# jhultman/vision3d

Measured on AMD Instinct MI355X. Metric: frames/sec SECOND fwd, 16k-pt KITTI cloud, higher is better.
Workload: dtype f16x3-scaled (fp32-class): fp32 operands split into f16 hi + lo pieces of x * s under per-tensor power-of-two scales, 3 MFMA terms (lo*hi + hi*lo + hi*hi), fp32 accumulate; relative product error 2^-22 -- the result differs from the reference's fp32 modules by fp32 summation noise: strict elementwis

## Files before the change

### vision3d_amd/csrc/spconv.hip

```cpp
#include "v3d_internal.h"

#include "sp_device.h"
#include "rb_device.h"

#define SP_RIDER_PROLOGUE(lds)                                                                        \
  if (rider.blocks && (int)blockIdx.x < rider.blocks) {                                               \
    if (threadIdx.x < V3D_BLOCK) rb_rider_run(rider, (int)blockIdx.x, (unsigned char*)(lds));         \
    return;                                                                                           \
  }                                                                                                   \
  const int bid = (int)blockIdx.x - rider.blocks;                                                     \
  [[maybe_unused]] const int nblk = (int)gridDim.x - rider.blocks;



__global__ __launch_bounds__(V3D_BLOCK) void spconv_fwd_scalar(const float* __restrict__ in,
                                                               const float* __restrict__ W,
                                                               const int* __restrict__ nbr,
                                                               const int* __restrict__ n_ptr, int cap, int K, int Cin,
                                                               int Cout, const float* __restrict__ scale,
                                                               const float* __restrict__ shift, int relu,
                                                               float* __restrict__ out) {
  const int n = min(*n_ptr, cap);
  const long long total = (long long)n * Cout;
  for (long long t = (long long)blockIdx.x * V3D_BLOCK + threadIdx.x; t < total; t += (long long)gridDim.x * V3D_BLOCK) {
    const int o = (int)(t / Cout), c = (int)(t % Cout);
    float acc = 0.f;
    for (int k = 0; k < K; k++) {
      const int i = nbr[(size_t)k * cap + o];
      if (i < 0) continue;
      const float* x = in + (size_t)i * Cin;
      const float* w = W + (size_t)k * Cin * Cout + c;
      float part = 0.f;
      for (int ci = 0; ci < Cin; ci++) part = fmaf(x[ci], w[(size_t)ci * Cout], part);
      acc += part;
    }
    if (scale) acc = acc * scale[c] + shift[c];
    if (relu) acc = fmaxf(acc, 0.f);
    out[t] = acc;
  }
}

#define SPC_TM 64

#define SPW_WAVES 8

template <int CIN, int COUT>
__global__ __launch_bounds__(SPW_WAVES* V3D_WAVE) void spconv_fwd_wave(const float* __restrict__ in,
                                                                       const float* __restrict__ W,
                                                                       const int* __restrict__ nbr,
                                                                       const int* __restrict__ n_ptr, int cap, int K,
                                                                       const float* __restrict__ scale,
                                                                       const float* __restrict__ shift, int relu,
                                                                       float* __restrict__ out, const float* __restrict__ next_entry,
                                                                       int* __restrict__ range_flag, unsigned* __restrict__ seen,
                                                                       const RbScanJob rider) {
  constexpr int NB = COUT / 16;
  constexpr int G = SPW_WAVES / NB;
  constexpr int T = CIN / 4;
  constexpr int NT = SPW_WAVES * V3D_WAVE;
  extern __shared__ __attribute__((aligned(16))) float smem[];
  float* acc = smem;
  int* list_in = (int*)(acc + G * SPC_TM * COUT);
  int* cnt_pad = list_in + K * SPC_TM;
  unsigned char* list_row = (unsigned char*)(cnt_pad + K);
  SP_RIDER_PROLOGUE(smem)

  const int n = min(*n_ptr, cap);
  const int row0 = bid * SPC_TM;
  if (row0 >= n) return;
  const int tid = threadIdx.x, lane = tid & 63, wave = tid >> 6;

  for (int i = tid; i < G * SPC_TM * COUT; i += NT) acc[i] = 0.f;
  for (int k = wave; k < K; k += SPW_WAVES) {
    const int row = row0 + lane;
    const int v = row < n ? nbr[(size_t)k * cap + row] : -1;
    const unsigned long long m = __ballot(v >= 0);
    const int c = __popcll(m);
    const int cp = (c + 15) & ~15;
    const int pos = __popcll(m & ((1ull << lane) - 1ull));
    if (v >= 0) {
      list_in[k * SPC_TM + pos] = v;
      list_row[k * SPC_TM + pos] = (unsigned char)lane;
    }
    if (lane >= c && lane < cp) {
      list_in[k * SPC_TM + lane] = -1;
      list_row[k * SPC_TM + lane] = 255;
    }
    if (lane == 0) cnt_pad[k] = cp;
  }
  __syncthreads();

  const int uwave = __builtin_amdgcn_readfirstlane(wave);
  const int g = uwave / NB, nb = uwave % NB;
  const int kper = (K + G - 1) / G;
  const int k_lo = g * kper, k_hi = min(K, k_lo + kper);
  const int r = lane & 15, q = lane >> 4;
  float* my_acc = acc + (size_t)g * SPC_TM * COUT + nb * 16 + r;
  const int cnt_reg = lane < K ? cnt_pad[lane] : 0;
  auto count_of = [&](int k) { return __builtin_amdgcn_readlane(cnt_reg, k); };

  float a0[T], a1[T], b0[T], b1[T];
  auto load_a = [&](int k, int rblk, float (&a)[T]) {
    const int src = list_in[k * SPC_TM + rblk * 16 + r];
    if (src >= 0) {
      const float* p = in + (size_t)src * CIN + q * T;
      if constexpr (T % 4 == 0) {
#pragma unroll
        for (int i = 0; i < T / 4; i++) {
          const float4 v = reinterpret_cast<const float4*>(p)[i];
          a[4 * i] = v.x;
          a[4 * i + 1] = v.y;
          a[4 * i + 2] = v.z;
          a[4 * i + 3] = v.w;
        }
      } else {
#pragma unroll
        for (int t = 0; t < T; t++) a[t] = p[t];
      }
    } else {
#pragma unroll
      for (int t = 0; t < T; t++) a[t] = 0.f;
    }
  };
  auto load_b = [&](int k, float (&b)[T]) {
    const float* p = W + ((size_t)k * CIN + q * T) * COUT + nb * 16 + r;
#pragma unroll
    for (int t = 0; t < T; t++) b[t] = p[(size_t)t * COUT];
  };
  auto advance = [&](int& k, int& rblk) {
    rblk++;
    if (rblk * 16 < count_of(k)) return;
    rblk = 0;
    do {
      k++;
    } while (k < k_hi && count_of(k) == 0);
  };

  int k = k_lo, rblk = 0;
  while (k < k_hi && count_of(k) == 0) k++;
  if (k < k_hi) {
    load_a(k, rblk, a0);
    load_b(k, b0);
  }
  while (k < k_hi) {
    int kn = k, rn = rblk;
    advance(kn, rn);
    const bool more = kn < k_hi, newk = kn != k;
    const unsigned rows4 = *reinterpret_cast<const unsigned*>(list_row + k * SPC_TM + rblk * 16 + q * 4);
    if (more) {
      load_a(kn, rn, a1);
      if (newk) load_b(kn, b1);
    }
    f32x4 d0 = {0.f, 0.f, 0.f, 0.f}, d1 = {0.f, 0.f, 0.f, 0.f};
    if constexpr (T >= 2) {
#pragma unroll
      for (int t = 0; t < T; t += 2) {
        d0 = __builtin_amdgcn_mfma_f32_16x16x4f32(a0[t], b0[t], d0, 0, 0, 0);
        d1 = __builtin_amdgcn_mfma_f32_16x16x4f32(a0[t + 1], b0[t + 1], d1, 0, 0, 0);
      }
      d0 += d1;
    } else {
      d0 = __builtin_amdgcn_mfma_f32_16x16x4f32(a0[0], b0[0], d0, 0, 0, 0);
    }
    {
      float old[4];
#pragma unroll
      for (int rr = 0; rr < 4; rr++) {
        const unsigned trow = (rows4 >> (8 * rr)) & 255u;
        old[rr] = trow != 255u ? my_acc[trow * COUT] : 0.f;
      }
#pragma unroll
      for (int rr = 0; rr < 4; rr++) {
        const unsigned trow = (rows4 >> (8 * rr)) & 255u;
        if (trow != 255u) my_acc[trow * COUT] = old[rr] + d0[rr];
      }
    }
    if (more) {
#pragma unroll
      for (int t = 0; t < T; t++) a0[t] = a1[t];
      if (newk) {
#pragma unroll
        for (int t = 0; t < T; t++) b0[t] = b1[t];
      }
    }
    k = kn;
    rblk = rn;
  }
  __syncthreads();

  float vmax = 0.f;
  for (int idx = tid; idx < SPC_TM * (COUT / 4); idx += NT) {
    const int rw = idx / (COUT / 4), c4 = idx % (COUT / 4);
    if (row0 + rw >= n) continue;
    float4 v = *reinterpret_cast<const float4*>(acc + rw * COUT + c4 * 4);
#pragma unroll
    for (int gg = 1; gg < G; gg++) {
      const float4 u = *reinterpret_cast<const float4*>(acc + ((size_t)gg * SPC_TM + rw) * COUT + c4 * 4);
      v.x += u.x;
      v.y += u.y;
      v.z += u.z;
      v.w += u.w;
    }
    if (scale) {
      const float4 sc = *reinterpret_cast<const float4*>(scale + c4 * 4);
      const float4 sh = *reinterpret_cast<const float4*>(shift + c4 * 4);
      v.x = v.x * sc.x + sh.x;
      v.y = v.y * sc.y + sh.y;
      v.z = v.z * sc.z + sh.z;
      v.w = v.w * sc.w + sh.w;
    }
    if (relu) {
      v.x = fmaxf(v.x, 0.f);
      v.y = fmaxf(v.y, 0.f);
      v.z = fmaxf(v.z, 0.f);
      v.w = fmaxf(v.w, 0.f);
    }
    vmax = fmaxf(fmaxf(vmax, fmaxf(fabsf(v.x), fabsf(v.y))), fmaxf(fabsf(v.z), fabsf(v.w)));
    *reinterpret_cast<float4*>(out + (size_t)(row0 + rw) * COUT + c4 * 4) = v;
  }
  if (next_entry && range_flag && vmax > next_entry[2]) atomicMax(range_flag, V3D_FLAG_RANGE);
  if (seen && next_entry) v3d_mark_seen(seen, vmax, next_entry[2] * (1.f / (float)(1 << V3D_QUIET_BITS)));
}

template <int CIN, int COUT>
static int launch_wave(const float* in, const float* W, const int* nbr, const int* n_ptr, int cap, int K,
                       const float* scale, const float* shift, int relu, float* out, hipStream_t st, const float* next_entry,
                       int* range_flag, unsigned* seen, const RbScanJob* rider, bool* rider_taken) {
  constexpr int G = SPW_WAVES / (COUT / 16);
  const size_t lds = std::max((size_t)G * SPC_TM * COUT * 4 + (size_t)K * SPC_TM * 4 + (size_t)K * 4 + (size_t)K * SPC_TM + 64, (size_t)RB_SCAN_LDS);
  if (lds > 64 * 1024) return V3D_EUNSUPPORTED;
  const RbScanJob r = rider ? *rider : RbScanJob{};
  hipLaunchKernelGGL((spconv_fwd_wave<CIN, COUT>), dim3(v3d_ceil_div(cap, SPC_TM) + r.blocks), dim3(SPW_WAVES * V3D_WAVE), lds, st,
                     in, W, nbr, n_ptr, cap, K, scale, shift, relu, out, next_entry, range_flag, seen, r);
  if (rider_taken) *rider_taken = r.blocks > 0;
  V3D_CHECK_LAUNCH();
  return V3D_OK;
}


template <int PREC>
__global__ void spconv_pack_weights_kernel(const float* __restrict__ W, int K, int Cin, int Cout, unsigned short* __restrict__ img) {
  const int KI = (Cin + 31) / 32, NB = Cout / 16;
  const long long total = (long long)K * KI * NB * 64 * 8;
  float sw = 1.f;
  if constexpr (PREC == 1) sw = v3d_wimg_weight_scale(reinterpret_cast<unsigned*>(img + total * 2));
  for (long long t = (long long)blockIdx.x * blockDim.x + threadIdx.x; t < total; t += (long long)gridDim.x * blockDim.x) {
    long long r = t;
    const int e = (int)(r % 8); r /= 8;
    const int lane = (int)(r % 64); r /= 64;
    const int nb = (int)(r % NB); r /= NB;
    const int ki = (int)(r % KI); r /= KI;
    const int k = (int)r;
    const int cin = ki * 32 + (lane >> 4) * 8 + e, cout = nb * 16 + (lane & 15);
    const float v = cin < Cin ? W[((size_t)k * Cin + cin) * Cout + cout] : 0.f;
    unsigned short h, l;
    split_one<PREC>(v, sw, h, l);
    const size_t base = ((((size_t)k * KI + ki) * NB + nb) * 2) * 512 + (size_t)lane * 8 + e;
    img[base] = h;
    img[base + 512] = l;
  }
}

__global__ void spconv_pack_batch_kernel(V3dPackJobs jobs) {
  const int j = blockIdx.y;
  const float* __restrict__ W = jobs.w[j];
  unsigned short* __restrict__ img = reinterpret_cast<unsigned short*>(jobs.img[j]);
  const int K = jobs.K[j], Cin = jobs.cin[j], Cout = jobs.cout[j], mode = jobs.mode[j];
  const int KI = (Cin + 31) / 32, NB = Cout / 16;
  const long long total = (long long)K * KI * NB * 64 * 8;
  for (long long t = (long long)blockIdx.x * blockDim.x + threadIdx.x; t < total; t += (long long)gridDim.x * blockDim.x) {
    long long r = t;
    const int e = (int)(r % 8); r /= 8;
    const int lane = (int)(r % 64); r /= 64;
    const int nb = (int)(r % NB); r /= NB;
    const int ki = (int)(r % KI); r /= KI;
    const int k = (int)r;
    const int cin = ki * 32 + (lane >> 4) * 8 + e, cout = nb * 16 + (lane & 15);
    float v = 0.f;
    if (cin < Cin) {
      if (mode == 0) v = W[((size_t)k * Cin + cin) * Cout + cout];
      else v = W[((size_t)(mode == 2 ? K - 1 - k : k) * Cout + cout) * Cin + cin];
    }
    unsigned short h, l;
    split_one<0>(v, 1.f, h, l);
    const size_t base = ((((size_t)k * KI + ki) * NB + nb) * 2) * 512 + (size_t)lane * 8 + e;
    img[base] = h;
    img[base + 512] = l;
  }
}

int v3d_i_sparse_conv_pack_batch(const V3dPackJobs& jobs, int n, hipStream_t stream) {
  if (n < 1 || n > V3D_PACK_JOBS_MAX) return V3D_EINVAL;
  for (int j = 0; j < n; j++)
    if (!jobs.w[j] || !jobs.img[j] || jobs.K[j] < 1 || jobs.cin[j] < 1 || jobs.cout[j] < 16 || jobs.cout[j] % 16) return V3D_EINVAL;
  hipLaunchKernelGGL(spconv_pack_batch_kernel, dim3(32, n), dim3(256), 0, stream, jobs);
  V3D_CHECK_LAUNCH();
  return V3D_OK;
}

__global__ __launch_bounds__(1024) void act_scale_from_rows_kernel(const float* __restrict__ rows, const int* __restrict__ n_ptr, int cap,
                                                                    int C, int headroom, float* __restrict__ entry) {
  __shared__ unsigned wmax[16];
  const long long total = (long long)(n_ptr ? min(*n_ptr, cap) : cap) * C;
  unsigned m = 0u;
  const long long vec = (((uintptr_t)rows & 15) == 0) ? total / 4 : 0;
  for (long long t = threadIdx.x; t < vec; t += 1024) {
    const uint4 v = reinterpret_cast<const uint4*>(rows)[t];
    m = max(max(m, v.x & 0x7FFFFFFFu), max(max(v.y & 0x7FFFFFFFu, v.z & 0x7FFFFFFFu), v.w & 0x7FFFFFFFu));
  }
  for (long long t = vec * 4 + threadIdx.x; t < total; t += 1024) m = max(m, __float_as_uint(rows[t]) & 0x7FFFFFFFu);
#pragma unroll
  for (int o = 32; o > 0; o >>= 1) m = max(m, (unsigned)__shfl_xor((int)m, o));
  if ((threadIdx.x & 63) == 0) wmax[threadIdx.x >> 6] = m;
  __syncthreads();
  if (threadIdx.x == 0) {
    for (int w = 1; w < 16; w++) m = max(m, wmax[w]);
    const float s = v3d_pow2_scale(m, V3D_F16S_ACT_TARGET - headroom);
    entry[0] = s;
    entry[1] = 1.f / s;
    entry[2] = 32768.f / s;
    entry[3] = __uint_as_float(m);
  }
}

#define V3D_ACT_SCALE_ITEMS 4096
__global__ __launch_bounds__(V3D_BLOCK) void act_scale_from_rows_grid_kernel(const float* __restrict__ rows, const int* __restrict__ n_ptr,
                                                                             int cap, int C, int headroom, float* __restrict__ entry,
                                                                             unsigned* __restrict__ scratch) {
  __shared__ unsigned wmax[V3D_BLOCK / V3D_WAVE];
  const long long total = (long long)(n_ptr ? min(*n_ptr, cap) : cap) * C;
  unsigned m = 0u;
  const long long vec = (((uintptr_t)rows & 15) == 0) ? total / 4 : 0;
  for (long long t = (long long)blockIdx.x * V3D_BLOCK + threadIdx.x; t < vec; t += (long long)gridDim.x * V3D_BLOCK) {
    const uint4 v = reinterpret_cast<const uint4*>(rows)[t];
    m = max(max(m, v.x & 0x7FFFFFFFu), max(max(v.y & 0x7FFFFFFFu, v.z & 0x7FFFFFFFu), v.w & 0x7FFFFFFFu));
  }
  for (long long t = vec * 4 + (long long)blockIdx.x * V3D_BLOCK + threadIdx.x; t < total; t += (long long)gridDim.x * V3D_BLOCK)
    m = max(m, __float_as_uint(rows[t]) & 0x7FFFFFFFu);
#pragma unroll
  for (int o = 32; o > 0; o >>= 1) m = max(m, (unsigned)__shfl_xor((int)m, o));
  if ((threadIdx.x & 63) == 0) wmax[threadIdx.x >> 6] = m;
  __syncthreads();
  if (threadIdx.x == 0) {
    for (int w = 1; w < V3D_BLOCK / V3D_WAVE; w++) m = max(m, wmax[w]);
    atomicMax(&scratch[0], m);
    __threadfence();
    if (atomicAdd(&scratch[1], 1u) == gridDim.x - 1) {
      __threadfence();
      m = atomicExch(&scratch[0], 0u);
      atomicExch(&scratch[1], 0u);
      const float s = v3d_pow2_scale(m, V3D_F16S_ACT_TARGET - headroom);
      entry[0] = s;
      entry[1] = 1.f / s;
      entry[2] = 32768.f / s;
      entry[3] = __uint_as_float(m);
    }
  }
}

extern "C" int v3d_act_scale_from_rows(const float* rows, const int32_t* n_rows, int cap, int C, int headroom_bits, float* entry,
                                        uint32_t* scratch, v3d_stream_t stream) {
  if (!rows || !entry || cap < 1 || C < 1 || headroom_bits < 0 || headroom_bits > 12) return V3D_EINVAL;
  if (!scratch) {
    hipLaunchKernelGGL(act_scale_from_rows_kernel, dim3(1), dim3(1024), 0, (hipStream_t)stream, rows, n_rows, cap, C, headroom_bits, entry);
  } else {
    const long long vec = ((long long)cap * C + 3) / 4;
    const int blocks = (int)std::min<long long>(512, std::max<long long>(1, (vec + V3D_ACT_SCALE_ITEMS - 1) / V3D_ACT_SCALE_ITEMS));
    hipLaunchKernelGGL(act_scale_from_rows_grid_kernel, dim3(blocks), dim3(V3D_BLOCK), 0, (hipStream_t)stream, rows, n_rows, cap, C,
                       headroom_bits, entry, scratch);
  }
  V3D_CHECK_LAUNCH();
  return V3D_OK;
}

extern "C" size_t v3d_sparse_conv_weight_image_bytes(int K, int Cin, int Cout) {
  return (size_t)K * ((Cin + 31) / 32) * (Cout / 16) * 2 * 512 * sizeof(unsigned short) + V3D_WIMG_TRAILER;
}

extern "C" int v3d_sparse_conv_pack_weights(const float* weight, int K, int Cin, int Cout, int prec, void* image,
                                             v3d_stream_t stream) {
  if (!weight || !image || K < 1 || Cin < 1 || Cout < 16 || Cout % 16) return V3D_EINVAL;
  if (prec != V3D_PREC_BF16X3 && prec != V3D_PREC_F16S) return V3D_EINVAL;
  hipStream_t st = (hipStream_t)stream;
  unsigned short* img = (unsigned short*)image;
  if (prec == V3D_PREC_F16S) {
    unsigned* trailer = reinterpret_cast<unsigned*>(reinterpret_cast<char*>(image) + v3d_sparse_conv_weight_image_bytes(K, Cin, Cout) - V3D_WIMG_TRAILER);
    V3D_CHECK_HIP(v3d_fill_async(trailer, 0, V3D_WIMG_TRAILER, st));
    hipLaunchKernelGGL(v3d_wmax_kernel<>, dim3(64), dim3(256), 0, st, weight, (const float*)nullptr, 1ll, (long long)K * Cin * Cout, trailer);
    hipLaunchKernelGGL(spconv_pack_weights_kernel<1>, dim3(256), dim3(256), 0, st, weight, K, Cin, Cout, img);
  } else {
    hipLaunchKernelGGL(spconv_pack_weights_kernel<0>, dim3(256), dim3(256), 0, st, weight, K, Cin, Cout, img);
  }
  V3D_CHECK_LAUNCH();
  return V3D_OK;
}

#ifndef SPR_TIMELINE
#define SPR_TIMELINE 0
#endif
#if SPR_TIMELINE
__device__ unsigned long long spr_tl[4][4][16];
extern "C" int v3d_debug_rows_timeline(unsigned long long* host_out) {
  return (int)hipMemcpyFromSymbol(host_out, HIP_SYMBOL(spr_tl), sizeof(spr_tl));
}
#define SPR_STAMP(idx) do { if (lane == 0 && wave < 4 && (blockIdx.x & 127) == 5 && blockIdx.x < 512) spr_tl[blockIdx.x >> 7][wave][idx] = __builtin_readcyclecounter(); } while (0)
#else
#define SPR_STAMP(idx)
#endif

template <int CIN, int COUT, int PREC, int INS>
__global__ __launch_bounds__(V3D_BLOCK) void spconv_fwd_rows(const float* __restrict__ in,
                                                             const unsigned short* __restrict__ wimg,
                                                             const int* __restrict__ nbr, const int* __restrict__ n_ptr,
                                                             int cap, int K, const float* __restrict__ scale,
                                                             const float* __restrict__ shift, int relu,
                                                             float* __restrict__ out, const V3dDensifyOut dn, const V3dActScale as,
                                                             unsigned short* __restrict__ out_s, const RbScanJob rider) {
  constexpr int KI = (CIN + 31) / 32, NB = COUT / 16;
  constexpr int NF = KI * NB * 2;
  constexpr int NW = V3D_BLOCK / V3D_WAVE;
  extern __shared__ __attribute__((aligned(16))) float smem_rows[];
  float* part = smem_rows;
  int* nbr_s = (int*)(part + NW * NB * 4 * 64);
  SP_RIDER_PROLOGUE(smem_rows)
  const int n = min(*n_ptr, cap);
  const int tid = threadIdx.x, lane = tid & 63;
  const int wave = __builtin_amdgcn_readfirstlane(tid >> 6);
  int wg = bid;
  {
    const int nwg = (n + 15) / 16;
    if (dn.hi && bid == 0 && tid == 0) *dn.pix_n = n;
    if (wg >= nwg) return;
    const int q = nwg / 8, rmd = nwg % 8, xcd = wg % 8, idx = wg / 8;
    wg = (xcd < rmd ? xcd * (q + 1) : rmd * (q + 1) + (xcd - rmd) * q) + idx;
  }
  const int row0 = wg * 16;
  const int r = lane & 15, kg = lane >> 4;
  const SpScales ss = sp_scales<PREC>(as, wimg, (size_t)K * NF * 512);
  SPR_STAMP(0);
  for (int k = tid >> 4; k < K; k += V3D_BLOCK / 16)
    nbr_s[k * 16 + r] = (row0 + r < n) ? nbr[(size_t)k * cap + row0 + r] : -1;
  __syncthreads();
  SPR_STAMP(1);

  float araw[2][KI][8];
  u32x4 braw[2][NF];
  auto load_ops = [&](int k, float (&a)[KI][8], u32x4 (&b)[NF]) {
    const int src = nbr_s[k * 16 + r];
#pragma unroll
    for (int ki = 0; ki < KI; ki++) {
      const int c0 = ki * 32 + kg * 8;
      if (src >= 0 && c0 < CIN) {
        const float* p = in + (size_t)src * CIN + c0;
        if constexpr (INS) {
          static_assert(!INS || CIN % 8 == 0, "split rows need whole 16-byte fragments");
          const char* q = reinterpret_cast<const char*>(in) + (size_t)src * CIN * 4 + c0 * 2;
          const float4 v0 = *reinterpret_cast<const float4*>(q), v1 = *reinterpret_cast<const float4*>(q + CIN * 2);
          a[ki][0] = v0.x; a[ki][1] = v0.y; a[ki][2] = v0.z; a[ki][3] = v0.w;
          a[ki][4] = v1.x; a[ki][5] = v1.y; a[ki][6] = v1.z; a[ki][7] = v1.w;
        } else if constexpr (CIN % 8 == 0) {
          const float4 v0 = reinterpret_cast<const float4*>(p)[0], v1 = reinterpret_cast<const float4*>(p)[1];
          a[ki][0] = v0.x; a[ki][1] = v0.y; a[ki][2] = v0.z; a[ki][3] = v0.w;
          a[ki][4] = v1.x; a[ki][5] = v1.y; a[ki][6] = v1.z; a[ki][7] = v1.w;
        } else {
#pragma unroll
          for (int e = 0; e < 8; e++) a[ki][e] = (c0 + e < CIN) ? p[e] : 0.f;
        }
      } else {
#pragma unroll
        for (int e = 0; e < 8; e++) a[ki][e] = 0.f;
      }
    }
    const u32x4* wp = reinterpret_cast<const u32x4*>(wimg) + (size_t)k * NF * 64 + lane;
#pragma unroll
    for (int f = 0; f < NF; f++) b[f] = wp[(size_t)f * 64];
  };

  f32x4 acc[NB];
#pragma unroll
  for (int j = 0; j < NB; j++) acc[j] = f32x4{0.f, 0.f, 0.f, 0.f};
  auto multiply = [&](const float (&a)[KI][8], const u32x4 (&b)[NF]) {
#pragma unroll
    for (int ki = 0; ki < KI; ki++) {
      u32x4 ah, al;
      split_in<PREC, INS>(a[ki], ss.s_in, ah, al);
#pragma unroll
      for (int j = 0; j < NB; j++) acc[j] = split_mfma<PREC>(al, b[(ki * NB + j) * 2], acc[j]);
#pragma unroll
      for (int j = 0; j < NB; j++) acc[j] = split_mfma<PREC>(ah, b[(ki * NB + j) * 2 + 1], acc[j]);
#pragma unroll
      for (int j = 0; j < NB; j++) acc[j] = split_mfma<PREC>(ah, b[(ki * NB + j) * 2], acc[j]);
    }
  };

  SPR_STAMP(2);
  if (wave < K) load_ops(wave, araw[0], braw[0]);
  SPR_STAMP(3);
  for (int k = wave; k < K; k += 2 * NW) {
    if (k + NW < K) load_ops(k + NW, araw[1], braw[1]);
    multiply(araw[0], braw[0]);
#if SPR_TIMELINE
    __builtin_amdgcn_sched_barrier(0);
    SPR_STAMP(4 + 2 * ((k - wave) / (2 * NW)));
#endif
    if (k + NW < K) {
      if (k + 2 * NW < K) load_ops(k + 2 * NW, araw[0], braw[0]);
      multiply(araw[1], braw[1]);
#if SPR_TIMELINE
      __builtin_amdgcn_sched_barrier(0);
      SPR_STAMP(5 + 2 * ((k - wave) / (2 * NW)));
#endif
    }
  }
#pragma unroll
  for (int j = 0; j < NB; j++)
#pragma unroll
    for (int rr = 0; rr < 4; rr++) part[((wave * NB + j) * 4 + rr) * 64 + lane] = acc[j][rr];
  SPR_STAMP(12);
  __syncthreads();
  SPR_STAMP(13);

  float vmax = 0.f;
  const float s_next = (PREC == 1 && (dn.hi || out_s)) ? as.next[0] : 1.f;
  unsigned char* stg_f = reinterpret_cast<unsigned char*>(nbr_s + K * 16);
  unsigned char* stg_s = stg_f + SP_STAGE_BYTES(COUT);
  for (int j = wave; j < NB; j += NW) {
    const int col = j * 16 + r;
    const float sc = (scale ? scale[col] : 1.f) * ss.undo, sh = scale ? shift[col] : 0.f;
#pragma unroll
    for (int rr = 0; rr < 4; rr++) {
      float v = part[((0 * NB + j) * 4 + rr) * 64 + lane];
#pragma unroll
      for (int w = 1; w < NW; w++) v += part[((w * NB + j) * 4 + rr) * 64 + lane];
      const int row = row0 + kg * 4 + rr;
      if (scale || PREC == 1) v = v * sc + sh;
      if (relu) v = fmaxf(v, 0.f);
      if (out) sp_stage_put_f32<COUT>(stg_f, kg * 4 + rr, col, v);
      if (out_s) sp_stage_put_split<PREC, COUT>(stg_s, kg * 4 + rr, col, r, v, s_next);
      if (row < n) {
        if constexpr (PREC == 1) vmax = fmaxf(vmax, fabsf(v));
        if (dn.hi) {
          const int4 c = reinterpret_cast<const int4*>(dn.coords)[row];
          const int pixel = (c.x * dn.H + c.z) * dn.W + c.w;
          const size_t o = (size_t)pixel * ((size_t)COUT * dn.D) + (size_t)col * dn.D + c.y;
          unsigned short h, l;
          split_one<PREC>(v, s_next, h, l);
          reinterpret_cast<unsigned short*>(dn.hi)[o] = h;
          reinterpret_cast<unsigned short*>(dn.lo)[o] = l;
          if (col == 0) {
            if (dn.occ) atomicAnd(dn.occ + ((size_t)c.x * dn.H + c.z) * ((dn.W + 31) >> 5) + (c.w >> 5), ~(1u << (c.w & 31)));
            dn.pix[row] = pixel;
          }
        }
      }
    }
  }
  if (out || out_s) {
    __syncthreads();
    const int nv = min(16, n - row0);
    if (out) sp_stage_flush<COUT, V3D_BLOCK>(stg_f, reinterpret_cast<unsigned char*>(out + (size_t)row0 * COUT), nv, tid);
    if (out_s) sp_stage_flush<COUT, V3D_BLOCK>(stg_s, reinterpret_cast<unsigned char*>(out_s + (size_t)row0 * (2 * COUT)), nv, tid);
  }
  if constexpr (PREC == 1) sp_range_check(as, vmax, ss.limit);
  SPR_STAMP(14);
}

template <int CIN, int COUT, int PREC, int INS>
__global__ __launch_bounds__(V3D_BLOCK) void spconv_fwd_rows_big(const float* __restrict__ in,
                                                                 const unsigned short* __restrict__ wimg,
                                                                 const int* __restrict__ nbr, const int* __restrict__ n_ptr,
                                                                 int cap, int K, const float* __restrict__ scale,
                                                                 const float* __restrict__ shift, int relu,
                                                                 float* __restrict__ out, const V3dActScale as,
                                                                 unsigned short* __restrict__ out_s) {
  constexpr int KI = (CIN + 31) / 32, NB = COUT / 16;
  constexpr int NF = KI * NB * 2;
  constexpr int WBYTES = NF * 64 * 16;
  constexpr int WLOADS = WBYTES / (V3D_BLOCK * 16);
  static_assert(WBYTES % (V3D_BLOCK * 16) == 0, "weight image must split evenly over the workgroup");
  extern __shared__ __attribute__((aligned(16))) float smem_rows[];
  unsigned char* wbuf = reinterpret_cast<unsigned char*>(smem_rows);
  int* nbr_s = reinterpret_cast<int*>(wbuf + 2 * WBYTES);
  const int n = min(*n_ptr, cap);
  const int tid = threadIdx.x, lane = tid & 63;
  const int wave = __builtin_amdgcn_readfirstlane(tid >> 6);
  const int row0 = blockIdx.x * 64;
  if (row0 >= n) return;
  const int r = lane & 15, kg = lane >> 4;
  const SpScales ss = sp_scales<PREC>(as, wimg, (size_t)K * NF * 512);
  for (int t = tid; t < K * 64; t += V3D_BLOCK) {
    const int k = t >> 6, rr = t & 63;
    nbr_s[t] = (row0 + rr < n) ? nbr[(size_t)k * cap + row0 + rr] : -1;
  }
  u32x4 wreg[WLOADS];
  auto load_w = [&](int k) {
    const u32x4* wp = reinterpret_cast<const u32x4*>(wimg) + (size_t)k * NF * 64 + tid;
#pragma unroll
    for (int i = 0; i < WLOADS; i++) wreg[i] = wp[(size_t)i * V3D_BLOCK];
  };
  auto store_w = [&](int buf) {
    u32x4* dst = reinterpret_cast<u32x4*>(wbuf + buf * WBYTES) + tid;
#pragma unroll
    for (int i = 0; i < WLOADS; i++) dst[(size_t)i * V3D_BLOCK] = wreg[i];
  };
  float araw[2][KI][8];
  auto load_a = [&](int k, float (&a)[KI][8]) {
    const int src = nbr_s[k * 64 + wave * 16 + r];
#pragma unroll
    for (int ki = 0; ki < KI; ki++) {
      const int c0 = ki * 32 + kg * 8;
      if (src >= 0 && c0 < CIN) {
        const char* p = reinterpret_cast<const char*>(in) + (size_t)src * CIN * 4 + (INS ? c0 * 2 : c0 * 4);
        const float4 v0 = *reinterpret_cast<const float4*>(p), v1 = *reinterpret_cast<const float4*>(p + (INS ? CIN * 2 : 16));
        a[ki][0] = v0.x; a[ki][1] = v0.y; a[ki][2] = v0.z; a[ki][3] = v0.w;
        a[ki][4] = v1.x; a[ki][5] = v1.y; a[ki][6] = v1.z; a[ki][7] = v1.w;
      } else {
#pragma unroll
        for (int e = 0; e < 8; e++) a[ki][e] = 0.f;
      }
    }
  };
  f32x4 acc[NB];
#pragma unroll
  for (int j = 0; j < NB; j++) acc[j] = f32x4{0.f, 0.f, 0.f, 0.f};
  auto multiply = [&](const float (&a)[KI][8], int buf) {
    const u32x4* bw = reinterpret_cast<const u32x4*>(wbuf + buf * WBYTES) + lane;
#pragma unroll
    for (int ki = 0; ki < KI; ki++) {
      u32x4 ah, al;
      split_in<PREC, INS>(a[ki], ss.s_in, ah, al);
#pragma unroll
      for (int j = 0; j < NB; j++) {
        const u32x4 bh = bw[(size_t)((ki * NB + j) * 2) * 64], bl = bw[(size_t)((ki * NB + j) * 2 + 1) * 64];
        acc[j] = split_mfma<PREC>(al, bh, acc[j]);
        acc[j] = split_mfma<PREC>(ah, bl, acc[j]);
        acc[j] = split_mfma<PREC>(ah, bh, acc[j]);
      }
    }
  };

  load_w(0);
  store_w(0);
  __syncthreads();
  load_a(0, araw[0]);
  for (int k = 0; k < K; k += 2) {
    if (k + 1 < K) {
      load_w(k + 1);
      load_a(k + 1, araw[1]);
    }
// ... 593 lines not shown
}

#define V3D_BIG_ROWS 32768
#define V3D_RING_ROWS 16384
template <int CIN, int COUT, int PREC, int INS>
static int launch_rows(const float* in, const void* wimg, const int* nbr, const int* n_ptr, int cap, int K,
                       const float* scale, const float* shift, int relu, float* out, int rows_hint, hipStream_t st,
                       const V3dDensifyOut* densify, int tiles_min, const SpLaunch& sl) {
  const int force = densify ? 1 : (rows_hint < 0 ? -rows_hint : 0);
  if constexpr (CIN >= 32 && CIN <= 64 && COUT >= 32 && COUT <= 64) {
    if (K == 27 && (force == 6 || force == 7 || force == 8 || (force == 0 && CIN == 64 && COUT == 64 && rows_hint >= V3D_BIG_ROWS))) {
      if (force == 7) launch_rows_kouter<CIN, COUT, 2, 0, PREC, INS>(in, wimg, nbr, n_ptr, cap, scale, shift, relu, out, st, sl);
      else if (force == 8) launch_rows_kouter<CIN, COUT, 2, 1, PREC, INS>(in, wimg, nbr, n_ptr, cap, scale, shift, relu, out, st, sl);
      else launch_rows_kouter<CIN, COUT, 3, 1, PREC, INS>(in, wimg, nbr, n_ptr, cap, scale, shift, relu, out, st, sl);
      V3D_CHECK_LAUNCH();
      return V3D_OK;
    }
    if (force == 5 || (force == 0 && rows_hint >= V3D_BIG_ROWS)) {
      launch_rows_big<CIN, COUT, PREC, INS>(in, wimg, nbr, n_ptr, cap, K, scale, shift, relu, out, st, sl);
      V3D_CHECK_LAUNCH();
      return V3D_OK;
    }
    if (K == 27 && (force == 10 || force == 16 || (force >= 12 && force <= 14) || (force == 0 && rows_hint <= V3D_RING_ROWS))) {
      if constexpr (CIN == 64 && COUT == 64) {
        if (force != 16) {
          const long long want = force ? 0 : (long long)rows_hint + rows_hint / 10;
          int tiles = force == 12 ? 2 : force == 13 ? 3 : force == 14 ? 4 : (want <= 32 * 256 ? 2 : want <= 48 * 256 ? 3 : 4);
          if (!force && tiles < tiles_min) tiles = tiles_min > 4 ? 4 : tiles_min;
          if (tiles == 2) return launch_rows_ring<CIN, COUT, 3, 2, 4, 1, 1, 2>(in, wimg, nbr, n_ptr, cap, scale, shift, relu, out, st, sl);
          if (tiles == 3) return launch_rows_ring<CIN, COUT, 3, 2, 4, 1, 1, 3>(in, wimg, nbr, n_ptr, cap, scale, shift, relu, out, st, sl);
          return launch_rows_ring<CIN, COUT, 3, 2, 4, 1, 1, 4>(in, wimg, nbr, n_ptr, cap, scale, shift, relu, out, st, sl);
        }
      }
      if (force != 16 && CIN == 32 && COUT == 32) return launch_rows_ring<CIN, COUT, 3, 2, 2, 2, 1>(in, wimg, nbr, n_ptr, cap, scale, shift, relu, out, st, sl);
      return launch_rows_ring<CIN, COUT, 3, 3, 2>(in, wimg, nbr, n_ptr, cap, scale, shift, relu, out, st, sl);
    }
  }
  const size_t lds = std::max((size_t)4 * (COUT / 16) * 4 * 64 * 4 + (size_t)K * 16 * 4 + 2 * SP_STAGE_BYTES(COUT),
                              (size_t)RB_SCAN_LDS);
  const RbScanJob r = sl.rider ? *sl.rider : RbScanJob{};
  hipLaunchKernelGGL((spconv_fwd_rows<CIN, COUT, PREC, INS>), dim3(v3d_ceil_div(cap, 16) + r.blocks), dim3(V3D_BLOCK), lds, st,
                     INS ? (const float*)sl.in_split : in, (const unsigned short*)wimg, nbr, n_ptr, cap, K, scale, shift, relu, out,
                     densify ? *densify : V3dDensifyOut{}, sl.as, sl.out_split, r);
  if (sl.rider_taken) *sl.rider_taken = r.blocks > 0;
  V3D_CHECK_LAUNCH();
  return V3D_OK;
}

extern "C" int v3d_sparse_conv_fwd_packed(const float* in, const void* weight_image, const int32_t* nbr,
                                           const int32_t* n_out, int cap_out, int K, int Cin, int Cout, const float* scale,
                                           const float* shift, int relu, float* out, int rows_hint, int prec,
                                           const float* act_in, const float* act_next, int32_t* range_flag,
                                           const void* in_split, void* out_split, v3d_stream_t stream) {
  const V3dActScale as{act_in, act_next, range_flag, nullptr};
  return v3d_i_sparse_conv_fwd_packed(in ? in : (const float*)in_split, weight_image, nbr, n_out, cap_out, K, Cin, Cout, scale, shift,
                                      relu, out, rows_hint, (hipStream_t)stream, nullptr, 2, prec, &as, in_split, out_split);
}

template <int PREC>
__global__ __launch_bounds__(256) void rows_split_kernel(const float* __restrict__ rows, const int* __restrict__ n_ptr, int cap, int C,
                                                         const float* __restrict__ entry, unsigned short* __restrict__ out) {
  const long long total = (long long)(n_ptr ? min(*n_ptr, cap) : cap) * C;
  const float s = PREC == 1 ? entry[0] : 1.f;
  for (long long t = (long long)blockIdx.x * 256 + threadIdx.x; t < total; t += (long long)gridDim.x * 256) {
    const long long row = t / C;
    const int c = (int)(t - row * C);
    unsigned short h, l;
    split_one<PREC>(rows[t], s, h, l);
    out[row * 2 * C + c] = h;
    out[row * 2 * C + C + c] = l;
  }
}

extern "C" int v3d_sparse_rows_split(const float* rows, const int32_t* n_rows, int cap, int C, int prec, const float* act_entry,
                                     void* out_split, v3d_stream_t stream) {
  if (!rows || !out_split || cap < 1 || C < 8 || C % 8) return V3D_EINVAL;
  if (prec == V3D_PREC_F16S ? !act_entry : prec != V3D_PREC_BF16X3) return V3D_EINVAL;
  const int blocks = (int)std::min<long long>(((long long)cap * C + 255) / 256, 4096);
  if (prec == V3D_PREC_F16S)
    hipLaunchKernelGGL(rows_split_kernel<1>, dim3(blocks), dim3(256), 0, (hipStream_t)stream, rows, n_rows, cap, C, act_entry, (unsigned short*)out_split);
  else
    hipLaunchKernelGGL(rows_split_kernel<0>, dim3(blocks), dim3(256), 0, (hipStream_t)stream, rows, n_rows, cap, C, nullptr, (unsigned short*)out_split);
  V3D_CHECK_LAUNCH();
  return V3D_OK;
}

bool v3d_i_sparse_conv_packed_supported(int Cin, int Cout) {
  static const int shapes[][2] = {{4, 16}, {16, 16}, {16, 32}, {32, 32}, {32, 64}, {64, 64}, {4, 32}, {32, 16}, {64, 32}, {64, 128}, {128, 128}};
  for (const auto& s : shapes)
    if (s[0] == Cin && s[1] == Cout) return true;
  return false;
}

int v3d_i_sparse_conv_fwd_packed(const float* in, const void* weight_image, const int32_t* nbr, const int32_t* n_out,
                                 int cap_out, int K, int Cin, int Cout, const float* scale, const float* shift, int relu,
                                 float* out, int rows_hint, hipStream_t st, const V3dDensifyOut* densify, int ring_tiles_min,
                                 int prec, const V3dActScale* act, const void* in_split, void* out_split, const RbScanJob* rider,
                                 bool* rider_taken) {
  if (rider_taken) *rider_taken = false;
  if (!in || !weight_image || !nbr || !n_out || (!out && !out_split) || cap_out < 1 || K < 1) return V3D_EINVAL;
  if ((scale == nullptr) != (shift == nullptr)) return V3D_EINVAL;
  if (!out && densify) return V3D_EINVAL;
  if (prec != V3D_PREC_BF16X3 && prec != V3D_PREC_F16S) return V3D_EINVAL;
  if (prec == V3D_PREC_F16S && (!act || !act->in || ((densify || out_split) && !act->next))) return V3D_EINVAL;
  if (in_split && Cin % 8) return V3D_EINVAL;
  SpLaunch sl;
  sl.prec = prec;
  sl.as = (prec == V3D_PREC_F16S) ? *act : V3dActScale{nullptr, nullptr, nullptr, nullptr};
  sl.in_split = in_split;
  sl.out_split = (unsigned short*)out_split;
  sl.rider = rider;
  sl.rider_taken = rider_taken;
#define V3D_GO(ci, co, P, I) \
  return launch_rows<ci, co, P, I>(in, weight_image, nbr, n_out, cap_out, K, scale, shift, relu, out, rows_hint, st, densify, ring_tiles_min, sl)
#define V3D_TRY(ci, co)                                    \
  if (Cin == ci && Cout == co) {                           \
    if constexpr ((ci) % 8 == 0) {                         \
      if (prec == V3D_PREC_F16S && in_split) V3D_GO(ci, co, 1, 1); \
      if (prec == V3D_PREC_BF16X3 && in_split) V3D_GO(ci, co, 0, 1); \
    }                                                      \
    if (prec == V3D_PREC_F16S) V3D_GO(ci, co, 1, 0);       \
    V3D_GO(ci, co, 0, 0);                                  \
  }
  V3D_TRY(4, 16)
  V3D_TRY(16, 16)
  V3D_TRY(16, 32)
  V3D_TRY(32, 32)
  V3D_TRY(32, 64)
  V3D_TRY(64, 64)
  V3D_TRY(4, 32)
  V3D_TRY(32, 16)
  V3D_TRY(64, 32)
  V3D_TRY(64, 128)
  V3D_TRY(128, 128)
#undef V3D_TRY
#undef V3D_GO
  return V3D_EUNSUPPORTED;
}

extern "C" int v3d_sparse_conv_fwd(const float* in, const float* weight, const int32_t* nbr, const int32_t* n_out,
                                   int cap_out, int K, int Cin, int Cout, const float* scale, const float* shift,
                                   int relu, float* out, int algo, v3d_stream_t stream) {
  return v3d_i_sparse_conv_fwd_exact(in, weight, nbr, n_out, cap_out, K, Cin, Cout, scale, shift, relu, out, algo, (hipStream_t)stream,
                                     nullptr, nullptr, nullptr, nullptr, nullptr);
}

int v3d_i_sparse_conv_fwd_exact(const float* in, const float* weight, const int32_t* nbr, const int32_t* n_out, int cap_out, int K,
                                int Cin, int Cout, const float* scale, const float* shift, int relu, float* out, int algo,
                                hipStream_t st, const float* next_entry, int32_t* range_flag, unsigned* seen, const RbScanJob* rider,
                                bool* rider_taken) {
  if (rider_taken) *rider_taken = false;
  if (!in || !weight || !nbr || !n_out || !out || cap_out < 1 || K < 1 || Cin < 1 || Cout < 1) return V3D_EINVAL;
  if ((scale == nullptr) != (shift == nullptr)) return V3D_EINVAL;
  if (algo != 0 && algo != 1 && algo != 3) return V3D_EINVAL;
  if (algo == 0 || algo == 3) {
    int rc = V3D_EUNSUPPORTED;
#define V3D_TRY(ci, co) \
  if (Cin == ci && Cout == co) rc = launch_wave<ci, co>(in, weight, nbr, n_out, cap_out, K, scale, shift, relu, out, st, next_entry, range_flag, seen, rider, rider_taken);
    V3D_TRY(4, 16)
    V3D_TRY(16, 16)
    V3D_TRY(16, 32)
    V3D_TRY(32, 32)
    V3D_TRY(32, 64)
    V3D_TRY(64, 64)
    V3D_TRY(4, 32)
    V3D_TRY(32, 16)
    V3D_TRY(64, 32)
    V3D_TRY(64, 128)
    V3D_TRY(128, 128)
#undef V3D_TRY
    if (rc != V3D_EUNSUPPORTED || algo == 3) return rc;
  }
  const long long total = (long long)cap_out * Cout;
  const int blocks = (int)((total + V3D_BLOCK - 1) / V3D_BLOCK);
  hipLaunchKernelGGL(spconv_fwd_scalar, dim3(blocks > 8192 ? 8192 : blocks), dim3(V3D_BLOCK), 0, st, in, weight, nbr,
                       n_out, cap_out, K, Cin, Cout, scale, shift, relu, out);
  V3D_CHECK_LAUNCH();
  return V3D_OK;
}

#define BW_MAX_SPLITS 64
#define BW_Q 128

__host__ __device__ static inline int bw_rows_per_block(int n) {
  const int r = ((n + BW_MAX_SPLITS - 1) / BW_MAX_SPLITS + 255) & ~255;
  return r < 256 ? 256 : r;
}

template <int TI, int TJ>
__global__ __launch_bounds__(V3D_BLOCK) void spconv_bwd_weight_tiles(const float* __restrict__ X,
                                                                     const float* __restrict__ dY,
                                                                     const int* __restrict__ nbr,
                                                                     const int* __restrict__ n_ptr, int cap, int Cin,
                                                                     int Cout, int groups_j,
                                                                     float* __restrict__ partial ) {
  __shared__ int q_src[4][BW_Q];
  __shared__ int q_out[4][BW_Q];
  __shared__ float red[TI * TJ * 256];
  const int n = min(*n_ptr, cap);
  const int rows_per_block = bw_rows_per_block(n);
  const int slab = blockIdx.x, k = blockIdx.y, K = gridDim.y;
  const int lo = slab * rows_per_block;
  if (lo >= n) return;
  const int hi = min(n, lo + rows_per_block);
  const int ci_base = (blockIdx.z / groups_j) * TI * 16, co_base = (blockIdx.z % groups_j) * TJ * 16;
  const int lane = threadIdx.x & 63, wave = threadIdx.x >> 6;
  const int r = lane & 15, p = lane >> 4;
  const int rows_per_wave = rows_per_block >> 2;
  const int wlo = lo + wave * rows_per_wave, whi = min(hi, wlo + rows_per_wave);
  const int* __restrict__ nk = nbr + (size_t)k * cap;
  int* qs = q_src[wave];
  int* qo = q_out[wave];

  f32x4 acc[TI][TJ];
#pragma unroll
  for (int t = 0; t < TI; t++)
#pragma unroll
    for (int u = 0; u < TJ; u++) acc[t][u] = f32x4{0.f, 0.f, 0.f, 0.f};

  auto consume = [&](int base, int valid) {
    float a[4][TI], b[4][TJ];
#pragma unroll
    for (int s4 = 0; s4 < 4; s4++) {
      const int e = 4 * s4 + p;
      const bool ok = e < valid;
      const int src = ok ? qs[base + e] : 0, o = ok ? qo[base + e] : 0;
#pragma unroll
      for (int t = 0; t < TI; t++) {
        const int ci = ci_base + 16 * t + r;
        a[s4][t] = (ok && ci < Cin) ? X[(size_t)src * Cin + ci] : 0.f;
      }
#pragma unroll
      for (int u = 0; u < TJ; u++) {
        const int co = co_base + 16 * u + r;
        b[s4][u] = (ok && co < Cout) ? dY[(size_t)o * Cout + co] : 0.f;
      }
    }
#pragma unroll
    for (int s4 = 0; s4 < 4; s4++)
#pragma unroll
      for (int t = 0; t < TI; t++)
#pragma unroll
        for (int u = 0; u < TJ; u++) acc[t][u] = __builtin_amdgcn_mfma_f32_16x16x4f32(a[s4][t], b[s4][u], acc[t][u], 0, 0, 0);
  };

  int cnt = 0;
  int src_next = (wlo < whi && wlo + lane < whi) ? nk[wlo + lane] : -1;
  for (int o0 = wlo; o0 < whi; o0 += 64) {
    const int src = src_next;
    const int o = o0 + lane;
    src_next = (o + 64 < whi) ? nk[o + 64] : -1;
    const unsigned long long live = __ballot(src >= 0);
    if (src >= 0) {
      const int pos = cnt + __popcll(live & ((1ull << lane) - 1ull));
      qs[pos] = src;
      qo[pos] = o;
    }
    cnt += __popcll(live);
    int g = 0;
    for (; cnt - g >= 16; g += 16) consume(g, 16);
    if (g) {
      const int rem = cnt - g;
      int ms = 0, mo = 0;
      if (lane < rem) { ms = qs[g + lane]; mo = qo[g + lane]; }
      if (lane < rem) { qs[lane] = ms; qo[lane] = mo; }
      cnt = rem;
    }
  }
  if (cnt > 0) consume(0, cnt);

  for (int w = 0; w < 4; w++) {
    if (wave == w) {
#pragma unroll
      for (int t = 0; t < TI; t++)
#pragma unroll
        for (int u = 0; u < TJ; u++)
#pragma unroll
          for (int rr = 0; rr < 4; rr++) {
            const int idx = (((t * TJ + u) * 4 + rr) << 6) + lane;
            red[idx] = w == 0 ? acc[t][u][rr] : red[idx] + acc[t][u][rr];
          }
    }
    __syncthreads();
  }
  float* outp = partial + ((size_t)slab * K + k) * Cin * Cout;
  for (int idx = threadIdx.x; idx < TI * TJ * 256; idx += V3D_BLOCK) {
    const int l = idx & 63, rr = (idx >> 6) & 3, tu = idx >> 8;
    const int ci = ci_base + 16 * (tu / TJ) + (l >> 4) * 4 + rr;
    const int co = co_base + 16 * (tu % TJ) + (l & 15);
    if (ci < Cin && co < Cout) outp[(size_t)ci * Cout + co] = red[idx];
  }
}

__global__ void spconv_bwd_weight_reduce_kernel(const float* __restrict__ partial, const int* __restrict__ n_ptr, int cap,
                                                long long elems, float* __restrict__ dW) {
  const int n = min(*n_ptr, cap);
  const int rows_per_block = bw_rows_per_block(n);
  const int slabs = (n + rows_per_block - 1) / rows_per_block;
  for (long long i = (long long)blockIdx.x * blockDim.x + threadIdx.x; i < elems; i += (long long)gridDim.x * blockDim.x) {
    float s = 0.f;
    for (int sp = 0; sp < slabs; sp++) s += partial[(size_t)sp * elems + i];
    dW[i] = s;
  }
}

extern "C" size_t v3d_sparse_conv_bwd_weight_workspace(int K, int Cin, int Cout) {
  return (size_t)BW_MAX_SPLITS * K * Cin * Cout * sizeof(float) + 256;
}

template <int TI, int TJ>
static void launch_bwd_weight(const float* X, const float* dY, const int* nbr, const int* n_out, int cap, int K, int Cin,
                              int Cout, int slabs, float* partial, hipStream_t st) {
  const int gi = ((Cin + 15) / 16 + TI - 1) / TI, gj = ((Cout + 15) / 16 + TJ - 1) / TJ;
  hipLaunchKernelGGL((spconv_bwd_weight_tiles<TI, TJ>), dim3(slabs, K, gi * gj), dim3(V3D_BLOCK), 0, st, X, dY, nbr, n_out,
                     cap, Cin, Cout, gj, partial);
}

extern "C" int v3d_sparse_conv_bwd_weight(const float* X, const float* dY, const int32_t* nbr, const int32_t* n_out,
                                          int cap_out, int K, int Cin, int Cout, float* dW, void* workspace,
                                          size_t workspace_bytes, v3d_stream_t stream) {
  hipStream_t st = (hipStream_t)stream;
  if (!X || !dY || !nbr || !n_out || !dW || !workspace || cap_out < 1 || K < 1 || K > 65535 || Cin < 1 || Cout < 1)
    return V3D_EINVAL;
  if (workspace_bytes < v3d_sparse_conv_bwd_weight_workspace(K, Cin, Cout)) return V3D_EWORKSPACE;
// ... 43 lines not shown
```

Measured before the change: 4795.

## Hoist all gather loads ahead of MFMA in small-channel sparse conv wave kernel

Adds a HOIST variant of the wave sparse-conv kernel for small channel counts. When each wave handles at most four kernel offsets, it issues every weight and neighbour-row gather up front, using buffer loads whose out-of-range offsets return zero, and only then runs the MFMA blocks. This replaces the serial double-buffered loop and is meant to remove the exposed load latency between blocks. A second change in the split-precision kernel issues the first weight load before the neighbour-table fill and barrier so it overlaps that setup. The hoisted path raises register use, and algo 5 is added to turn hoisting off.

```diff
diff --git a/vision3d_amd/csrc/spconv.hip b/vision3d_amd/csrc/spconv.hip
--- a/vision3d_amd/csrc/spconv.hip
+++ b/vision3d_amd/csrc/spconv.hip
@@ -44,7 +44,14 @@
 
 #define SPW_WAVES 8
 
+#define SPW_HOIST_K 4
 template <int CIN, int COUT>
+constexpr bool spw_hoist_ok() {
+  constexpr int G = SPW_WAVES / (COUT / 16);
+  return (CIN / 4) * 4 * ((27 + G - 1) / G) <= 16;
+}
+
+template <int CIN, int COUT, bool HOIST>
 __global__ __launch_bounds__(SPW_WAVES* V3D_WAVE) void spconv_fwd_wave(const float* __restrict__ in,
                                                                        const float* __restrict__ W,
                                                                        const int* __restrict__ nbr,
@@ -136,55 +143,87 @@
     } while (k < k_hi && count_of(k) == 0);
   };
 
-  int k = k_lo, rblk = 0;
-  while (k < k_hi && count_of(k) == 0) k++;
-  if (k < k_hi) {
-    load_a(k, rblk, a0);
-    load_b(k, b0);
-  }
-  while (k < k_hi) {
-    int kn = k, rn = rblk;
-    advance(kn, rn);
-    const bool more = kn < k_hi, newk = kn != k;
+  auto block = [&](int k, int rblk, const float (&a)[T], const float (&b)[T]) {
     const unsigned rows4 = *reinterpret_cast<const unsigned*>(list_row + k * SPC_TM + rblk * 16 + q * 4);
-    if (more) {
-      load_a(kn, rn, a1);
-      if (newk) load_b(kn, b1);
-    }
     f32x4 d0 = {0.f, 0.f, 0.f, 0.f}, d1 = {0.f, 0.f, 0.f, 0.f};
     if constexpr (T >= 2) {
 #pragma unroll
       for (int t = 0; t < T; t += 2) {
-        d0 = __builtin_amdgcn_mfma_f32_16x16x4f32(a0[t], b0[t], d0, 0, 0, 0);
-        d1 = __builtin_amdgcn_mfma_f32_16x16x4f32(a0[t + 1], b0[t + 1], d1, 0, 0, 0);
+        d0 = __builtin_amdgcn_mfma_f32_16x16x4f32(a[t], b[t], d0, 0, 0, 0);
+        d1 = __builtin_amdgcn_mfma_f32_16x16x4f32(a[t + 1], b[t + 1], d1, 0, 0, 0);
       }
       d0 += d1;
     } else {
-      d0 = __builtin_amdgcn_mfma_f32_16x16x4f32(a0[0], b0[0], d0, 0, 0, 0);
-    }
-    {
-      float old[4];
-#pragma unroll
-      for (int rr = 0; rr < 4; rr++) {
-        const unsigned trow = (rows4 >> (8 * rr)) & 255u;
-        old[rr] = trow != 255u ? my_acc[trow * COUT] : 0.f;
-      }
-#pragma unroll
-      for (int rr = 0; rr < 4; rr++) {
-        const unsigned trow = (rows4 >> (8 * rr)) & 255u;
-        if (trow != 255u) my_acc[trow * COUT] = old[rr] + d0[rr];
-      }
-    }
-    if (more) {
-#pragma unroll
-      for (int t = 0; t < T; t++) a0[t] = a1[t];
-      if (newk) {
-#pragma unroll
-        for (int t = 0; t < T; t++) b0[t] = b1[t];
-      }
-    }
-    k = kn;
-    rblk = rn;
+      d0 = __builtin_amdgcn_mfma_f32_16x16x4f32(a[0], b[0], d0, 0, 0, 0);
+    }
+    float old[4];
+#pragma unroll
+    for (int rr = 0; rr < 4; rr++) {
+      const unsigned trow = (rows4 >> (8 * rr)) & 255u;
+      old[rr] = trow != 255u ? my_acc[trow * COUT] : 0.f;
+    }
+#pragma unroll
+    for (int rr = 0; rr < 4; rr++) {
+      const unsigned trow = (rows4 >> (8 * rr)) & 255u;
+      if (trow != 255u) my_acc[trow * COUT] = old[rr] + d0[rr];
+    }
+  };
+
+  if constexpr (HOIST) {
+    float ah[SPW_HOIST_K][4][T], bh[SPW_HOIST_K][T];
+    int cnt[SPW_HOIST_K], src[SPW_HOIST_K][4];
+#pragma unroll
+    for (int i = 0; i < SPW_HOIST_K; i++) {
+      const int kc = min(k_lo + i, K - 1);
+      cnt[i] = k_lo + i < k_hi ? count_of(kc) : 0;
+      load_b(kc, bh[i]);
+#pragma unroll
+      for (int rb = 0; rb < 4; rb++) {
+        const int e = list_in[kc * SPC_TM + rb * 16 + r];
+        src[i][rb] = rb * 16 < cnt[i] ? e : -1;
+      }
+    }
+    const __amdgpu_buffer_rsrc_t rows_rs = __builtin_amdgcn_make_buffer_rsrc(const_cast<float*>(in), 0, 0x7FFFFFFF, 0x00020000);
+#pragma unroll
+    for (int i = 0; i < SPW_HOIST_K; i++)
+#pragma unroll
+      for (int rb = 0; rb < 4; rb++) {
+        const unsigned off = src[i][rb] >= 0 ? ((unsigned)src[i][rb] * CIN + q * T) * 4 : 0x80000000u;
+#pragma unroll
+        for (int t = 0; t < T; t++) ah[i][rb][t] = __uint_as_float(__builtin_amdgcn_raw_buffer_load_b32(rows_rs, off + 4 * t, 0, 0));
+      }
+#pragma unroll
+    for (int i = 0; i < SPW_HOIST_K; i++)
+#pragma unroll
+      for (int rb = 0; rb < 4; rb++)
+        if (rb * 16 < cnt[i]) block(k_lo + i, rb, ah[i][rb], bh[i]);
+  } else {
+    int k = k_lo, rblk = 0;
+    while (k < k_hi && count_of(k) == 0) k++;
+    if (k < k_hi) {
+      load_a(k, rblk, a0);
+      load_b(k, b0);
+    }
+    while (k < k_hi) {
+      int kn = k, rn = rblk;
+      advance(kn, rn);
+      const bool more = kn < k_hi, newk = kn != k;
+      if (more) {
+        load_a(kn, rn, a1);
+        if (newk) load_b(kn, b1);
+      }
+      block(k, rblk, a0, b0);
+      if (more) {
+#pragma unroll
+        for (int t = 0; t < T; t++) a0[t] = a1[t];
+        if (newk) {
+#pragma unroll
+          for (int t = 0; t < T; t++) b0[t] = b1[t];
+        }
+      }
+      k = kn;
+      rblk = rn;
+    }
   }
   __syncthreads();
 
@@ -225,12 +264,15 @@
 template <int CIN, int COUT>
 static int launch_wave(const float* in, const float* W, const int* nbr, const int* n_ptr, int cap, int K,
                        const float* scale, const float* shift, int relu, float* out, hipStream_t st, const float* next_entry,
-                       int* range_flag, unsigned* seen, const RbScanJob* rider, bool* rider_taken) {
+                       int* range_flag, unsigned* seen, const RbScanJob* rider, bool* rider_taken, bool hoist) {
   constexpr int G = SPW_WAVES / (COUT / 16);
   const size_t lds = std::max((size_t)G * SPC_TM * COUT * 4 + (size_t)K * SPC_TM * 4 + (size_t)K * 4 + (size_t)K * SPC_TM + 64, (size_t)RB_SCAN_LDS);
   if (lds > 64 * 1024) return V3D_EUNSUPPORTED;
   const RbScanJob r = rider ? *rider : RbScanJob{};
-  hipLaunchKernelGGL((spconv_fwd_wave<CIN, COUT>), dim3(v3d_ceil_div(cap, SPC_TM) + r.blocks), dim3(SPW_WAVES * V3D_WAVE), lds, st,
+  auto kern = spconv_fwd_wave<CIN, COUT, false>;
+  if constexpr (spw_hoist_ok<CIN, COUT>())
+    if (hoist && K <= SPW_HOIST_K * G) kern = spconv_fwd_wave<CIN, COUT, true>;
+  hipLaunchKernelGGL(kern, dim3(v3d_ceil_div(cap, SPC_TM) + r.blocks), dim3(SPW_WAVES * V3D_WAVE), lds, st,
                      in, W, nbr, n_ptr, cap, K, scale, shift, relu, out, next_entry, range_flag, seen, r);
   if (rider_taken) *rider_taken = r.blocks > 0;
   V3D_CHECK_LAUNCH();
@@ -438,14 +480,20 @@
   const int r = lane & 15, kg = lane >> 4;
   const SpScales ss = sp_scales<PREC>(as, wimg, (size_t)K * NF * 512);
   SPR_STAMP(0);
+  float araw[2][KI][8];
+  u32x4 braw[2][NF];
+  auto load_b = [&](int k, u32x4 (&b)[NF]) {
+    const u32x4* wp = reinterpret_cast<const u32x4*>(wimg) + (size_t)k * NF * 64 + lane;
+#pragma unroll
+    for (int f = 0; f < NF; f++) b[f] = wp[(size_t)f * 64];
+  };
+  if (wave < K) load_b(wave, braw[0]);
   for (int k = tid >> 4; k < K; k += V3D_BLOCK / 16)
     nbr_s[k * 16 + r] = (row0 + r < n) ? nbr[(size_t)k * cap + row0 + r] : -1;
   __syncthreads();
   SPR_STAMP(1);
 
-  float araw[2][KI][8];
-  u32x4 braw[2][NF];
-  auto load_ops = [&](int k, float (&a)[KI][8], u32x4 (&b)[NF]) {
+  auto load_a = [&](int k, float (&a)[KI][8]) {
     const int src = nbr_s[k * 16 + r];
 #pragma unroll
     for (int ki = 0; ki < KI; ki++) {
@@ -471,9 +519,10 @@
         for (int e = 0; e < 8; e++) a[ki][e] = 0.f;
       }
     }
-    const u32x4* wp = reinterpret_cast<const u32x4*>(wimg) + (size_t)k * NF * 64 + lane;
-#pragma unroll
-    for (int f = 0; f < NF; f++) b[f] = wp[(size_t)f * 64];
+  };
+  auto load_ops = [&](int k, float (&a)[KI][8], u32x4 (&b)[NF]) {
+    load_a(k, a);
+    load_b(k, b);
   };
 
   f32x4 acc[NB];
@@ -494,7 +543,7 @@
   };
 
   SPR_STAMP(2);
-  if (wave < K) load_ops(wave, araw[0], braw[0]);
+  if (wave < K) load_a(wave, araw[0]);
   SPR_STAMP(3);
   for (int k = wave; k < K; k += 2 * NW) {
     if (k + NW < K) load_ops(k + NW, araw[1], braw[1]);
@@ -1394,11 +1443,11 @@
   if (rider_taken) *rider_taken = false;
   if (!in || !weight || !nbr || !n_out || !out || cap_out < 1 || K < 1 || Cin < 1 || Cout < 1) return V3D_EINVAL;
   if ((scale == nullptr) != (shift == nullptr)) return V3D_EINVAL;
-  if (algo != 0 && algo != 1 && algo != 3) return V3D_EINVAL;
-  if (algo == 0 || algo == 3) {
+  if (algo != 0 && algo != 1 && algo != 3 && algo != 5) return V3D_EINVAL;
+  if (algo == 0 || algo == 3 || algo == 5) {
     int rc = V3D_EUNSUPPORTED;
 #define V3D_TRY(ci, co) \
-  if (Cin == ci && Cout == co) rc = launch_wave<ci, co>(in, weight, nbr, n_out, cap_out, K, scale, shift, relu, out, st, next_entry, range_flag, seen, rider, rider_taken);
+  if (Cin == ci && Cout == co) rc = launch_wave<ci, co>(in, weight, nbr, n_out, cap_out, K, scale, shift, relu, out, st, next_entry, range_flag, seen, rider, rider_taken, algo != 5);
     V3D_TRY(4, 16)
     V3D_TRY(16, 16)
     V3D_TRY(16, 32)
@@ -1411,7 +1460,7 @@
     V3D_TRY(64, 128)
     V3D_TRY(128, 128)
 #undef V3D_TRY
-    if (rc != V3D_EUNSUPPORTED || algo == 3) return rc;
+    if (rc != V3D_EUNSUPPORTED || algo == 3 || algo == 5) return rc;
   }
   const long long total = (long long)cap_out * Cout;
   const int blocks = (int)((total + V3D_BLOCK - 1) / V3D_BLOCK);
```

After: 4803, median of 6. Within noise of the previous version (+0.2%).
